# chaiyujin/sdfa-2019

Hardware: AMD Instinct MI355X
Metric: animation frames/s/node (10 s@16 kHz clips); max|Δdgrad| vs CPU ref (higher is better)
Workload: dtype f32

## Files before the change

sdfa-2019_amd/csrc/api_core.cpp:

```cpp
#include "../../include/sdfa_stream.h"
#include "host.h"

#include <climits>
#include <cstdio>
#include <cstring>
#include <string>

static thread_local std::string g_err;

int sdfa_failv(int code, const char *fmt, va_list ap) {
    char buf[512];
    vsnprintf(buf, sizeof buf, fmt, ap);
    g_err = buf;
    return code;
}

int sdfa_fail(int code, const char *fmt, ...) {
    va_list ap;
    va_start(ap, fmt);
    sdfa_failv(code, fmt, ap);
    va_end(ap);
    return code;
}

thread_local int g_sdfa_mel_fft_radix4 = 0;
thread_local int g_sdfa_gather_plain_order = 0;
thread_local int g_sdfa_frontend_two_kernel = 0;
thread_local int g_sdfa_frontend_stream_block = 0;
thread_local int g_sdfa_frontend_stream_slots = 0;
thread_local int g_sdfa_frontend_stream_spin_max = 0;
thread_local int g_sdfa_frontend_stream_phases = 0;
thread_local int g_sdfa_frontend_t_major = 0;
extern thread_local int g_sdfa_gemm_variant;
thread_local int g_sdfa_freq_lstm_shape = 0;
thread_local int g_sdfa_pca_lds = 0;
thread_local int g_sdfa_pca_fp32 = 0;
thread_local int g_sdfa_conv_fp32 = 0;
thread_local int g_sdfa_time_lstm_split = 0;
thread_local int g_sdfa_time_lstm_fuse_x = 0;
thread_local int g_sdfa_time_lstm_handoff = 0;
thread_local int g_sdfa_time_lstm_timeout_us = 0;
thread_local int g_sdfa_share_gx0_off = 0;
thread_local int g_sdfa_encoder_dedup_off = 0;
thread_local int g_sdfa_share_hash_bits = 0;
thread_local int g_sdfa_freq_proj_tail = 0;
thread_local int g_sdfa_attn_unfused = 0;

extern "C" {

int sdfa_abi_version(void) { return SDFA_ABI_VERSION; }
int sdfa_stream_abi_version(void) { return SDFA_STREAM_ABI_VERSION; }
const char *sdfa_last_error(void) { return g_err.c_str(); }

int sdfa_debug_set_option(const char *name, int value) {
    struct Option { const char *name; int *var; int lo = INT_MIN, hi = INT_MAX; const char *accepts = nullptr; };
    thread_local const Option options[] = {
        {"attn_unfused", &g_sdfa_attn_unfused},
        {"share_gx0_off", &g_sdfa_share_gx0_off},
        {"encoder_dedup_off", &g_sdfa_encoder_dedup_off},
        {"share_hash_bits", &g_sdfa_share_hash_bits, 0, 32, "0 (the whole hash) or 1..32 low bits"},
        {"freq_proj_tail", &g_sdfa_freq_proj_tail, 0, 2, "0 (rule), 1 (never) or 2 (always)"},
        {"frontend_two_kernel", &g_sdfa_frontend_two_kernel},
        {"frontend_stream_phases", &g_sdfa_frontend_stream_phases},
        {"frontend_stream_spin_max", &g_sdfa_frontend_stream_spin_max, 0, INT_MAX, "0 (default) or a positive poll count"},
        {"frontend_stream_block", &g_sdfa_frontend_stream_block, 0, 256, "0 (default) or 1..256 frames"},
        {"frontend_stream_slots", &g_sdfa_frontend_stream_slots, 0, 256, "0 (default) or 1..256 workgroups per block"},
        {"gather_plain_order", &g_sdfa_gather_plain_order},
        {"mel_fft_radix4", &g_sdfa_mel_fft_radix4},
        {"frontend_t_major", &g_sdfa_frontend_t_major},
        {"time_lstm_timeout_us", &g_sdfa_time_lstm_timeout_us},
        {"time_lstm_handoff", &g_sdfa_time_lstm_handoff},
        {"time_lstm_split", &g_sdfa_time_lstm_split},
        {"time_lstm_fuse_x", &g_sdfa_time_lstm_fuse_x, 0, 3, "0 (rule), 1 (never), 2 or 3 (always, 32- / 64-frame tiles)"},
        {"gemm_variant", &g_sdfa_gemm_variant},
        {"freq_lstm_shape", &g_sdfa_freq_lstm_shape},
        {"pca_lds", &g_sdfa_pca_lds},
        {"conv_fp32", &g_sdfa_conv_fp32},
        {"pca_fp32", &g_sdfa_pca_fp32},
    };
    for (const Option &o : options)
        if (name && !strcmp(name, o.name)) {
            if (value < o.lo || value > o.hi) return sdfa_fail(SDFA_EINVAL, "%s: %s", o.name, o.accepts);
            *o.var = value;
            return SDFA_OK;
        }
    return sdfa_fail(SDFA_EINVAL, "unknown option '%s'", name ? name : "(null)");
}

}
```

sdfa-2019_amd/csrc/api_forward.cpp:

```cpp
#include "common.h"
#include "host.h"
#include "kernels.h"
#include "model.h"

#include <algorithm>

extern thread_local int g_sdfa_gemm_variant, g_sdfa_freq_lstm_shape, g_sdfa_pca_lds, g_sdfa_pca_fp32, g_sdfa_conv_fp32, g_sdfa_share_gx0_off, g_sdfa_attn_unfused, g_sdfa_encoder_dedup_off,
    g_sdfa_freq_proj_tail, g_sdfa_share_hash_bits;

namespace {

constexpr int64_t CT_WORDS = 2048, CT_FLAGS = 16, ST_WORDS = SDFA_WS_STATUS_BYTES / 4;

struct Ws {
    int64_t P1, X3, HF, Z, GX, H0, H1, KP, QC, QP, ZK, SH, ZU, total;
    int64_t TRUNK, A0, A1, COEF;
    int64_t CT_FREQ, CT_PCA, CT_FLAG;
};

Ws layout(int64_t Nc, bool keep) {
    const int64_t Mc = 64 * Nc;
    Ws w{};
    int64_t o = 0;
    auto take = [&](int64_t n) { int64_t r = o; o += round_up(n, 64); return r; };
    take(ST_WORDS);
    if (keep) {
        w.P1 = take(2048 * Mc); w.X3 = take(2048 * Mc); w.HF = take((int64_t)HF_SLAB_ROWS * 4 * Mc); w.Z = take(256 * Mc);
        w.GX = take(2048 * Mc); w.H0 = take(512 * Mc); w.H1 = take(512 * Mc); w.KP = take(128 * Mc);
    } else {
        const int64_t A = take(2048 * Mc);
        const int64_t B = take(2048 * Mc);
        w.HF = take((int64_t)HF_SLAB_ROWS * 4 * Mc);
        w.P1 = A; w.GX = A;
        w.X3 = B; w.Z = B; w.H0 = B + 256 * Mc; w.H1 = B + 768 * Mc; w.KP = B + 1280 * Mc;
    }
    w.QC = take(512 * Nc); w.QP = take(128 * Nc); w.ZK = take(512 * Nc);
    const int64_t R = take(2560 * Nc);
    w.TRUNK = R; w.A0 = R + 512 * Nc; w.A1 = R + 1024 * Nc; w.COEF = R + 1280 * Nc;
    w.SH = take(sdfa_share_table_words(Nc) + 111);
    w.ZU = keep ? take(256 * Mc) : w.P1;
    const int64_t CT = take(CT_WORDS);
    w.CT_FREQ = CT; w.CT_PCA = CT + 1; w.CT_FLAG = CT + CT_FLAGS;
    w.total = o;
    return w;
}

int64_t capacity(int64_t bytes, bool keep) {
    const int64_t per128 = layout(128, keep).total * 4;
    int64_t nc = (bytes / per128 + 2) * 128;
    while (nc > 0 && layout(nc, keep).total * 4 > bytes) nc -= 128;
    return nc;
}

struct Prof {
    const sdfa_model *m;
    hipStream_t s;
    hipEvent_t pending = nullptr;
    void begin(const char *stage) {
        if (!m->profile) return;
        sdfa_model::Ev e; e.stage = stage;
        (void)hipEventCreate(&e.a); (void)hipEventCreate(&e.b);
        (void)hipEventRecord(e.a, s);
        pending = e.b;
        std::lock_guard<std::mutex> lk(m->ev_mu);
        m->events.push_back(e);
    }
    void end() {
        if (!m->profile || !pending) return;
        (void)hipEventRecord(pending, s);
        pending = nullptr;
    }
};

GemmArgs gemm_fc(const sdfa_model::Fc &fc, const float *Q, int64_t ldq, float *D, int64_t Nc, const int64_t *spk, int64_t nreal) {
    GemmArgs g = sdfa_gemm_k4(fc.w, fc.Ppad, Q, ldq, D, Nc, fc.K);
    g.bias = fc.b; g.cond_w = fc.cw; g.cond_idx = fc.cw ? spk : nullptr;
    g.Pstore = fc.Pstore; g.Qreal = nreal; g.act = fc.act;
    return g;
}

}

extern "C" {

int64_t sdfa_workspace_bytes(const sdfa_model *m, int64_t max_frames) {
    if (!m || max_frames <= 0) return sdfa_fail(SDFA_EINVAL, "workspace_bytes: bad argument");
    return layout(round_up(max_frames, 128), m->keep).total * 4;
}

int sdfa_debug_keep_intermediates(sdfa_model *m, int on) {
    if (!m) return sdfa_fail(SDFA_EINVAL, "null model");
    m->keep = on != 0;
    return SDFA_OK;
}

int sdfa_profile_enable(sdfa_model *m, int on) {
    if (!m) return sdfa_fail(SDFA_EINVAL, "null model");
    std::lock_guard<std::mutex> lk(m->ev_mu);
    m->profile = on != 0;
    for (auto &e : m->events) { (void)hipEventDestroy(e.a); (void)hipEventDestroy(e.b); }
    m->events.clear();
    return SDFA_OK;
}

float sdfa_profile_ms(const sdfa_model *m, const char *stage) {
    if (!m || !stage) return (float)sdfa_fail(SDFA_EINVAL, "profile_ms: bad argument");
    float total = 0.f;
    bool any = false;
    std::lock_guard<std::mutex> lk(m->ev_mu);
    for (auto &e : m->events)
        if (e.stage == stage) {
            float ms = 0.f;
            if (hipEventSynchronize(e.b) != hipSuccess || hipEventElapsedTime(&ms, e.a, e.b) != hipSuccess)
                return (float)sdfa_fail(SDFA_EHIP, "profile_ms: event query failed");
            total += ms; any = true;
        }
    return any ? total : (float)sdfa_fail(SDFA_EINVAL, "profile_ms: no such stage '%s'", stage);
}

int sdfa_profile_reset(sdfa_model *m) { return m ? sdfa_profile_enable(m, m->profile) : sdfa_fail(SDFA_EINVAL, "null model"); }

enum { STAGE_BODY = 0, STAGE_ATTENTION = 1, STAGE_REGRESSOR = 2 };
static int stage_terms(const sdfa_model *m, int stage) {
    switch (m->precision) {
    case SDFA_PREC_BF16_ATTENTION: return stage == STAGE_ATTENTION ? 1 : 0;
    case SDFA_PREC_BF16X3_ATTENTION: return stage == STAGE_ATTENTION ? 3 : 0;
    case SDFA_PREC_BF16X6: return 6;
    case SDFA_PREC_BF16X3: return 3;
    case SDFA_PREC_BF16: return 1;
    default: return 0;
    }
}

int sdfa_model_set_precision(sdfa_model *m, int mode) {
    if (!m) return sdfa_fail(SDFA_EINVAL, "null model");
    if (mode < SDFA_PREC_FP32 || mode > SDFA_PREC_BF16X6) return sdfa_fail(SDFA_EINVAL, "unknown precision mode %d", mode);
    m->precision = mode;
    return SDFA_OK;
}

int sdfa_model_precision(const sdfa_model *m) { return m ? m->precision : SDFA_EINVAL; }

int sdfa_model_set_reserved_cus(sdfa_model *m, int k) {
    if (!m) return sdfa_fail(SDFA_EINVAL, "null model");
    if (k < 0 || k > 128) return sdfa_fail(SDFA_EINVAL, "reserved_cus must be in [0, 128], got %d", k);
    m->reserved_cus.store(k);
    return SDFA_OK;
}

static int encoder_impl(const sdfa_model *m, const float *d_audio_feat, int64_t n_frames, const int32_t *d_frame_clip,
                        const int64_t *d_frame_start, int hop, float *d_z, float *d_align, void *d_workspace,
                        int64_t workspace_bytes, void *stream) {
    if (!m || !m->finalized) return sdfa_fail(SDFA_ESTATE, "encoder_forward: model not finalised");
    if (n_frames == 0) return SDFA_OK;
    if (!d_audio_feat || !d_z || !d_workspace || n_frames < 0) return sdfa_fail(SDFA_EINVAL, "encoder_forward: bad argument");
    if (((uintptr_t)d_workspace | (uintptr_t)d_audio_feat | (uintptr_t)d_z) & 15) return sdfa_fail(SDFA_EINVAL, "encoder_forward: pointers must be 16-byte aligned");
    if ((uintptr_t)d_align & 3) return sdfa_fail(SDFA_EINVAL, "encoder_forward: d_align must be 4-byte aligned");
    const int64_t cap = capacity(workspace_bytes, m->keep);
    if (cap < 128) return sdfa_fail(SDFA_ENOSPACE, "encoder_forward: workspace of %lld bytes holds no 128-frame chunk", (long long)workspace_bytes);
    hipStream_t s = (hipStream_t)stream;
    Prof pf{m, s};
    float *ws = (float *)d_workspace;
    for (int64_t f0 = 0; f0 < n_frames; f0 += cap) {
        const int64_t N = std::min(cap, n_frames - f0);
        const int64_t Nc = round_up(N, 128), Mc = 64 * Nc;
        const Ws w = layout(Nc, m->keep);
        ConvArgs ca{};
        ca.audio_feat = d_audio_feat + f0 * (64 * 128 * 3); ca.N = N; ca.Nc = Nc; ca.Mc = Mc;
        ca.w1 = m->w1; ca.b1 = m->b1; ca.s1 = m->s1; ca.t1 = m->t1; ca.P1 = ws + w.P1;
        ca.w2 = m->w2; ca.b2 = m->b2; ca.s2 = m->s2; ca.t2 = m->t2;
        ca.w3 = m->w3; ca.b3 = m->b3; ca.s3 = m->s3; ca.t3 = m->t3; ca.X3 = ws + w.X3;
        const bool table = d_frame_clip != nullptr;
        const bool share = table || (!m->keep && !g_sdfa_encoder_dedup_off);
        const int64_t *d_ulimit = nullptr;
        int32_t *col_to_u = nullptr;
        bool split_tail = false;
        int64_t fat_grid = 0;
        const int64_t *d_qfull = nullptr;
        if (share) {
            ShareArgs sa{};
            sa.N = N; sa.Nc = Nc; sa.Mc = Mc;
            sdfa_share_carve(sa, reinterpret_cast<int32_t *>(ws + w.SH));
            split_tail = !m->keep && stage_terms(m, STAGE_BODY) == 0 && g_sdfa_gemm_variant == 0 && Mc / 256 >= 512 && g_sdfa_freq_proj_tail != 1;
            if (split_tail) {
                fat_grid = sdfa_fat_grid(256, Mc, sdfa_cu_count(), m->reserved_cus.load());
                sa.fat_grid = (int)fat_grid; sa.tail_mode = g_sdfa_freq_proj_tail;
            }
            pf.begin("share_map");
            if (table) {
                sa.frame_clip = d_frame_clip + f0; sa.frame_start = d_frame_start + f0; sa.hop = hop;
                sa.t_lo = 6; sa.t_hi = 58;
                HIP_TRY(sdfa_launch_share_map(sa, s));
            } else {
                sa.feat = ca.audio_feat;
                sa.hash = reinterpret_cast<uint64_t *>(ws + w.HF);
                sa.group_slots = sdfa_share_group_slots(N);
                sa.group_key = sa.hash + Mc; sa.group_first = reinterpret_cast<uint32_t *>(sa.group_key + sa.group_slots);
                sa.hash_bits = g_sdfa_share_hash_bits;
                HIP_TRY(sdfa_launch_share_map_content(sa, s));
            }
            pf.end();
            d_ulimit = sa.counts + 1; d_qfull = sa.counts + 2; col_to_u = sa.col_to_u;
            ca.col_src = sa.col_src; ca.col_limit = d_ulimit;
        }
        const int conv_terms = g_sdfa_conv_fp32 ? 0 : stage_terms(m, STAGE_BODY);
        if (m->keep && conv_terms) {
            pf.begin("conv1"); HIP_TRY(sdfa_launch_conv1(ca, s)); pf.end();
            ca.wb = m->cv_wb; ca.terms = conv_terms;
            pf.begin("conv23"); HIP_TRY(sdfa_launch_conv123(ca, s)); pf.end();
        } else if (m->keep) {
            pf.begin("conv1"); HIP_TRY(sdfa_launch_conv1(ca, s)); pf.end();
            pf.begin("conv23"); HIP_TRY(sdfa_launch_conv23(ca, s)); pf.end();
        } else {
            ca.wb = m->cv_wb; ca.terms = conv_terms;
            pf.begin("conv23"); HIP_TRY(sdfa_launch_conv123(ca, s)); pf.end();
        }

        const int fl_terms = stage_terms(m, STAGE_BODY);
        FreqLstmArgs fa{ws + w.X3, m->fl_w, m->fl_b, ws + w.HF, Mc, d_ulimit, m->fl_wb, fl_terms, reinterpret_cast<int *>(ws + w.CT_FREQ),
                        g_sdfa_freq_lstm_shape ? g_sdfa_freq_lstm_shape : (fl_terms ? 0 : m->freq_shape.load()), m->reserved_cus.load()};
        pf.begin("freq_lstm"); HIP_TRY(sdfa_launch_freq_lstm(fa, s)); pf.end();

        GemmArgs g = sdfa_gemm_k4(m->fp_w, 256, ws + w.HF, Mc, ws + w.Z, Mc, 8192);
        g.bias = m->fp_b; g.q_tile_major = 1; g.q_slab_rows = HF_SLAB_ROWS;
        g.terms = stage_terms(m, STAGE_BODY);
        g.reserve_cus = m->reserved_cus.load();
        if (share) { g.D = ws + w.ZU; g.q_limit = split_tail ? d_qfull : d_ulimit; }
        pf.begin("freq_proj");
        HIP_TRY(sdfa_launch_gemm(g, s));
        if (split_tail) {
            GemmTailArgs gt{m->fp_w, ws + w.HF, m->fp_b, ws + w.ZU, Mc, HF_SLAB_ROWS, d_qfull, d_ulimit, (int)fat_grid - 1};
            HIP_TRY(sdfa_launch_gemm_tail(gt, s));
        }
        pf.end();
        const bool share_gx0 = share && !m->keep && stage_terms(m, STAGE_BODY) == 0 && !g_sdfa_share_gx0_off;
        if (share && !share_gx0) {
            pf.begin("share_expand"); HIP_TRY(sdfa_launch_expand_cols(ws + w.ZU, col_to_u, ws + w.Z, 64, Mc, s)); pf.end();
        }

        const float *xin = share_gx0 ? ws + w.ZU : ws + w.Z;
        float *hout[2] = {ws + w.H0, ws + w.H1};
        const char *gxn[2] = {"gx0", "gx1"}, *lsn[2] = {"lstm0", "lstm1"};
        for (int l = 0; l < 2; ++l) {
            const bool mapped = share_gx0 && l == 0;
            float *gx = mapped ? ws + w.HF : ws + w.GX;
            GemmArgs gi = sdfa_gemm_k4(m->gx_w[l], 2048, xin, Mc, gx, Mc, l == 0 ? 256 : 512);
            gi.terms = stage_terms(m, STAGE_BODY);
            gi.reserve_cus = m->reserved_cus.load();
            if (mapped) gi.q_limit = d_ulimit;
            TimeLstmArgs ta{gx, m->tl_w[l], hout[l], Nc, Mc, m->tl_wb[l], stage_terms(m, STAGE_BODY),
                            reinterpret_cast<unsigned *>(ws + w.CT_FLAG), CT_WORDS - CT_FLAGS, m->tl_w16[l],
                            reinterpret_cast<unsigned *>(ws), m->reserved_cus.load(), mapped ? col_to_u : nullptr};
            if (l == 1 && !m->keep) { ta.X = xin; ta.Wxh = m->tl_wxh1; }
            pf.begin(gxn[l]);
            if (!sdfa_time_lstm_fuses_x(ta)) HIP_TRY(sdfa_launch_gemm(gi, s));
            pf.end();
            pf.begin(lsn[l]); HIP_TRY(sdfa_launch_time_lstm(ta, s)); pf.end();
            xin = hout[l];
        }
        const int at_terms = stage_terms(m, STAGE_ATTENTION);
        const bool key_fused = g_sdfa_attn_unfused != 1;
        pf.begin("attn_proj");
        GemmArgs gk = sdfa_gemm_k4(m->kp_w, 128, ws + w.H1, Mc, ws + w.KP, Mc, 512);
        gk.terms = at_terms;
        if (!key_fused) HIP_TRY(sdfa_launch_gemm(gk, s));
        GemmArgs gc = sdfa_gemm_k4(m->qc_w, 512, ws + w.H1 + 31 * Nc * 4, Mc, ws + w.QC, Nc, 1536);
        gc.seg_k = 512; gc.seg_col = Nc; gc.terms = at_terms;
        HIP_TRY(sdfa_launch_gemm(gc, s));
        GemmArgs gq = sdfa_gemm_k4(m->qp_w, 128, ws + w.QC, Nc, ws + w.QP, Nc, 512);
        gq.terms = at_terms;
        HIP_TRY(sdfa_launch_gemm(gq, s));
        const bool tail_fused = key_fused && (at_terms == 0 || at_terms == 6) && g_sdfa_attn_unfused != 2 && sdfa_attn_fuses_tail(Nc, m->reserved_cus.load());
        if (key_fused) {
            AttnKeyArgs ak{};
            ak.Wk = m->kp_w; ak.H = ws + w.H1; ak.QP = ws + w.QP; ak.v = m->at_v; ak.b = m->at_b;
            ak.S = ws + w.KP;
            ak.Nc = Nc; ak.Mc = Mc; ak.terms = at_terms == 6 ? 0 : at_terms; ak.reserve_cus = m->reserved_cus.load();
            if (tail_fused) {
                ak.fuse_tail = 1; ak.Zk4 = ws + w.ZK; ak.z_out = d_z + f0 * 512; ak.align_out = d_align ? d_align + f0 * 64 : nullptr; ak.N = N;
            }
            HIP_TRY(sdfa_launch_attn_key_score(ak, s));
        }
        pf.end();

        AttnArgs aa{};
        aa.KP = ws + w.KP; aa.QP = ws + w.QP; aa.H = ws + w.H1; aa.v = m->at_v; aa.b = m->at_b;
        aa.Zk4 = ws + w.ZK; aa.z_out = d_z + f0 * 512; aa.align_out = d_align ? d_align + f0 * 64 : nullptr;
        aa.N = N; aa.Nc = Nc; aa.Mc = Mc;
        aa.S = key_fused ? ws + w.KP : nullptr;
        pf.begin("attn"); if (!tail_fused) HIP_TRY(sdfa_launch_attn(aa, s)); pf.end();
    }
    return SDFA_OK;
}

int sdfa_model_autotune(sdfa_model *m, int64_t n_frames, void *d_workspace, int64_t workspace_bytes, void *stream) {
    if (!m || !m->finalized) return sdfa_fail(SDFA_ESTATE, "autotune: model not finalised");
    if (!d_workspace || n_frames <= 0 || ((uintptr_t)d_workspace & 15)) return sdfa_fail(SDFA_EINVAL, "autotune: bad argument");
    const int64_t cap = capacity(workspace_bytes, m->keep);
    if (cap < 128) return sdfa_fail(SDFA_ENOSPACE, "autotune: workspace too small");
    const int64_t Nc = round_up(std::min(cap, n_frames), 128), Mc = 64 * Nc;
    const Ws w = layout(Nc, m->keep);
    float *ws = (float *)d_workspace;
    hipStream_t s = (hipStream_t)stream;
    HIP_TRY(hipMemsetAsync(ws + w.X3, 0, (size_t)2048 * Mc * sizeof(float), s));
    hipEvent_t e0, e1;
    HIP_TRY(hipEventCreate(&e0));
    HIP_TRY(hipEventCreate(&e1));
    static const int forms[] = {9, 8, 5, 3};
    float best_ms = 0.f;
    int best = m->freq_shape.load(), rc = SDFA_OK;
    for (int form : forms) {
        FreqLstmArgs fa{ws + w.X3, m->fl_w, m->fl_b, ws + w.HF, Mc, nullptr, m->fl_wb, 0, reinterpret_cast<int *>(ws + w.CT_FREQ), form, m->reserved_cus.load()};
        float ms = 0.f;
        for (int rep = 0; rep < 3 && rc == SDFA_OK; ++rep) {
            if (rep == 1 && hipEventRecord(e0, s) != hipSuccess) rc = SDFA_EHIP;
            if (sdfa_launch_freq_lstm(fa, s) != hipSuccess) rc = SDFA_EHIP;
        }
        if (rc == SDFA_OK && (hipEventRecord(e1, s) != hipSuccess || hipEventSynchronize(e1) != hipSuccess || hipEventElapsedTime(&ms, e0, e1) != hipSuccess)) rc = SDFA_EHIP;
        if (rc != SDFA_OK) break;
        if (best_ms == 0.f || ms < best_ms) { best_ms = ms; best = form; }
    }
    (void)hipEventDestroy(e0);
    (void)hipEventDestroy(e1);
    if (rc != SDFA_OK) return sdfa_fail(rc, "autotune: a HIP call failed: %s", hipGetErrorString(hipGetLastError()));
    m->freq_shape.store(best);
    return best;
}

int sdfa_encoder_forward(const sdfa_model *m, const float *d_audio_feat, int64_t n_frames, float *d_z, float *d_align,
                         void *d_workspace, int64_t workspace_bytes, void *stream) {
    return encoder_impl(m, d_audio_feat, n_frames, nullptr, nullptr, 0, d_z, d_align, d_workspace, workspace_bytes, stream);
}

int sdfa_encoder_forward_shared(const sdfa_model *m, const float *d_audio_feat, int64_t n_frames, const int32_t *d_frame_clip,
                                const int64_t *d_frame_start, int hop, float *d_z, float *d_align, void *d_workspace,
                                int64_t workspace_bytes, void *stream) {
    if (!d_frame_clip || !d_frame_start || hop <= 0) return sdfa_fail(SDFA_EINVAL, "encoder_forward_shared: frame table missing");
    return encoder_impl(m, d_audio_feat, n_frames, d_frame_clip, d_frame_start, hop, d_z, d_align, d_workspace, workspace_bytes, stream);
}

static hipError_t expand_rows(const sdfa_model *m, const float *coef, int64_t N, int64_t Nc, int64_t f0,
                              float *const *h_d_outs, int n_outs, int *queue, hipStream_t s) {
    float *d_out = h_d_outs[0];
    if (m->pca_n == 2) {
        PcaArgs pa{};
        pa.coef = coef; pa.basis_s = m->pca_q[0]; pa.basis_r = m->pca_q[1]; pa.mean_s = m->pca_bias[0]; pa.mean_r = m->pca_bias[1];
        pa.out = d_out + f0 * m->out_dim; pa.N = N; pa.Nc = Nc; pa.out_dim = m->out_dim;
        pa.n_extra = n_outs - 1;
        pa.reserve_cus = m->reserved_cus.load();
        pa.basis_b = m->pca_qb; pa.terms = (g_sdfa_pca_fp32 || m->precision != SDFA_PREC_BF16X3) ? 0 : 3;
        for (int x = 1; x < n_outs; ++x) pa.out_extra[x - 1] = h_d_outs[x] + f0 * m->out_dim;
// ... 162 lines not shown
```

sdfa-2019_amd/csrc/kernels.h:

```cpp
#pragma once
#include <hip/hip_runtime.h>
#include <stdint.h>

enum { ACT_NONE = 0, ACT_LRELU = 1, ACT_TANH = 2 };

constexpr int HF_SLAB_ROWS = 2048;
enum { OUT_K4 = 0, OUT_ROW = 1 };
constexpr int SDFA_MAX_DESTS = 8;

struct GemmArgs {
    const float *P;
    const float *Q;
    float *D;
    const float *bias;
    const float *cond_w;
    const int64_t *cond_idx;
    int64_t ldp, ldq, ldd;
    int64_t Ppad, Qpad;
    int64_t Pstore;
    int64_t Qreal;
    int K;
    int seg_k;
    int64_t seg_col;
    int act, out_mode, bias_on_q;
// ... 12 lines not shown
    g.P = P; g.Q = Q; g.D = D;
    g.ldp = rows; g.Ppad = rows; g.Pstore = rows;
    g.ldq = ldq; g.ldd = cols; g.Qpad = cols; g.Qreal = cols;
    g.K = K; g.seg_k = K; g.act = ACT_NONE; g.out_mode = OUT_K4;
    return g;
}

struct PcaArgs {
    const float *coef;
    const float *basis_s, *basis_r;
    const float *mean_s, *mean_r;
    float *out;
    int64_t N, Nc, out_dim, ld_s, ld_r, cols_s, cols_r;
    float *out_extra[SDFA_MAX_DESTS - 1];
    int n_extra;
    int reserve_cus;
    const void *basis_b;
    int terms;
};
hipError_t sdfa_launch_pca_dgrad(const PcaArgs &a, hipStream_t s);
hipError_t sdfa_launch_pca_dgrad_res(const PcaArgs &a, int *queue, hipStream_t s);

struct FrontendConsts {
    const float *hamm;
    const float2 *twiddle;
    const int *mel_bin0;
    const float *mel_w8;
    int win, hop, sliding, nbins_used, nnz;
};
hipError_t sdfa_launch_frontend(const FrontendConsts &c, const float *pcm, const int64_t *clip_off,
                                const int64_t *clip_len, const int32_t *frame_clip, const int64_t *frame_start,
                                int64_t n_frames, float *audio_feat, hipStream_t s);
hipError_t sdfa_launch_mel_columns(const FrontendConsts &c, const float *pcm, const int64_t *clip_off, const int64_t *clip_len,
                                   const int32_t *frame_clip, const int64_t *frame_start, const int32_t *col_src,
                                   const int64_t *n_distinct, float *mel_table, hipStream_t s);
hipError_t sdfa_launch_mel_stream(const FrontendConsts &c, const float *pcm, const int64_t *clip_off, const int64_t *clip_len,
                                  const int32_t *frame_clip, const int64_t *frame_start, const int32_t *prev, const int32_t *shift,
                                  int64_t n_frames, int block, int slots, int producer_consumer, int spin_max, int *status, float *audio_feat, hipStream_t s);
hipError_t sdfa_launch_mel_ring(const FrontendConsts &c, const float *rings, int r, int n_rings, const int64_t *view_ring, const int64_t *view_hi,
                                const int32_t *frame_view, const int64_t *frame_start, const int32_t *prev, const int32_t *shift, int64_t n_frames,
                                int block, int slots, int producer_consumer, int spin_max, int *status, float *audio_feat, hipStream_t s);
hipError_t sdfa_launch_ring_append(float *rings, int r, int n_rings, const int64_t *seg, int n_seg, const float *src, int64_t n_src, hipStream_t s);
hipError_t sdfa_launch_gather_features(const float *mel_table, const int32_t *col_to_u, int64_t n_frames, int64_t Nc, int frame_major,
                                       float *audio_feat, hipStream_t s);

struct ConvArgs {
    const float *audio_feat;
    int64_t N, Nc, Mc;
    const float *w1, *b1, *s1, *t1;
    float *P1;
    const float *w2, *b2, *s2, *t2;
    const float *w3, *b3, *s3, *t3;
    float *X3;
    const int32_t *col_src;
    const int64_t *col_limit;
    const void *wb;
    int terms;
};
hipError_t sdfa_launch_conv1(const ConvArgs &a, hipStream_t s);
hipError_t sdfa_launch_conv23(const ConvArgs &a, hipStream_t s);
hipError_t sdfa_launch_conv123(const ConvArgs &a, hipStream_t s);

struct FreqLstmArgs {
    const float *X3;
    const float *W;
    const float *bias;
    float *HF;
    int64_t Mc;
    const int64_t *col_limit;
    const void *Wb;
    int terms;
    int *tile_counter;
    int shape;
    int reserve_cus;
};
hipError_t sdfa_launch_freq_lstm(const FreqLstmArgs &a, hipStream_t s);

struct TimeLstmArgs {
    const float *GX;
    const float *W;
    float *H;
    int64_t Nc, Mc;
    const void *Wb;
    int terms;
    unsigned *flags;
    int64_t flag_words;
    const float *W16;
    unsigned *status;
    int reserve_cus;
    const int32_t *col_map;
    const float *X = nullptr;
    const float *Wxh = nullptr;
};
hipError_t sdfa_launch_time_lstm(const TimeLstmArgs &a, hipStream_t s);
int sdfa_time_lstm_fuses_x(const TimeLstmArgs &a);

struct AttnArgs {
    const float *KP;
    const float *QP;
    const float *H;
    const float *v;
    const float *b;
    float *Zk4;
    float *z_out;
    float *align_out;
    int64_t N, Nc, Mc;
    const float *S;
};
hipError_t sdfa_launch_attn(const AttnArgs &a, hipStream_t s);

struct AttnKeyArgs {
    const float *Wk;
    const float *H;
    const float *QP;
    const float *v, *b;
    float *S;
    int64_t Nc, Mc;
    int terms;
    int reserve_cus;
    int ts_shift;
    int fuse_tail;
    float *Zk4, *z_out, *align_out;
    int64_t N;
};
bool sdfa_attn_fuses_tail(int64_t Nc, int reserve_cus);
hipError_t sdfa_launch_attn_key_score(const AttnKeyArgs &a, hipStream_t s);

hipError_t sdfa_launch_rows_to_k4(const float *src, int64_t N, int F, float *dst, int64_t ld, hipStream_t s);
hipError_t sdfa_launch_rows_seg_to_k4(const float *src, int64_t src_ld, int64_t N, int c0, int nf, float *dst, int64_t ld,
                                      int f0, int nf_pad, hipStream_t s);
hipError_t sdfa_launch_k4_to_rows(const float *src, int64_t ld, int64_t N, int F, int f0, int nf, float *dst,
                                  int64_t dst_ld, hipStream_t s);
hipError_t sdfa_launch_tap(const float *src, int what, int64_t N, int64_t Nc, float *dst, hipStream_t s);

struct ShareArgs {
    const int32_t *frame_clip;
    const int64_t *frame_start;
    int hop;
    int t_lo, t_hi;
    int frame_major;
    int64_t N, Nc, Mc;
    int32_t *prev, *shift;
    int32_t *owner, *flag, *uid;
    int32_t *tile_sum;
    int32_t *col_src;
    int32_t *col_to_u;
    int64_t *counts;
    const float *feat;
    uint64_t *hash;
    uint64_t *group_key;
    uint32_t *group_first;
    int64_t group_slots;
    int hash_bits;
    int fat_grid;
    int tail_mode;
};
inline int64_t sdfa_share_table_words(int64_t Nc) { return 16 + 2 * Nc + 5 * (64 * Nc) + (64 * Nc) / 1024 + 1; }
inline int64_t sdfa_share_group_slots(int64_t N) { int64_t s = 1024; while (s < 2 * 64 * N) s <<= 1; return s; }
inline void sdfa_share_carve(ShareArgs &a, int32_t *base) {
    a.counts = reinterpret_cast<int64_t *>(base);
    a.prev = base + 16; a.shift = a.prev + a.Nc;
    a.owner = a.shift + a.Nc; a.flag = a.owner + a.Mc; a.uid = a.flag + a.Mc;
    a.col_src = a.uid + a.Mc; a.col_to_u = a.col_src + a.Mc; a.tile_sum = a.col_to_u + a.Mc;
}
hipError_t sdfa_launch_share_map(const ShareArgs &a, hipStream_t s);
hipError_t sdfa_launch_share_map_content(const ShareArgs &a, hipStream_t s);
hipError_t sdfa_launch_share_prev(const ShareArgs &a, hipStream_t s);
hipError_t sdfa_launch_expand_cols(const float *Zu, const int32_t *col_to_u, float *Z, int nquads, int64_t Mc, hipStream_t s);

struct GemmTailArgs {
    const float *P, *Q, *bias;
    float *D;
    int64_t ldd;
    int q_slab_rows;
    const int64_t *q_lo, *q_hi;
    int max_tiles;
};
hipError_t sdfa_launch_gemm_tail(const GemmTailArgs &a, hipStream_t s);
inline int64_t sdfa_fat_grid(int64_t rows, int64_t cols, int cus, int reserve_cus) {
    const int64_t ntiles = (rows / 256) * (cols / 256), wgs = cus - reserve_cus > 1 ? cus - reserve_cus : 1;
    return ntiles < wgs ? ntiles : wgs;
}

struct MeshArgs {
    const float *dgrad;
    int64_t n_frames;
    int n_tris, n_verts, n_free, free_pad;
    int n_src_tris;
    const int64_t *seek_src;
    const float *seek_w;
    const float *reg_xt;
    const int *inc_ptr;
    const int *inc_tri;
    const float *inc_coef;
    const int *vert_col;
    const float *tmpl;
    float *rhs;
    const float *sol;
    float *verts;
    int64_t ld;
};
hipError_t sdfa_launch_mesh_rhs(const MeshArgs &a, hipStream_t s);
hipError_t sdfa_launch_mesh_scatter(const MeshArgs &a, hipStream_t s);
hipError_t sdfa_launch_seek_plan(const int32_t *tslist, const int64_t *frame_off, const int64_t *query_off, int n_clips, double fps,
                                 int64_t n_queries, int64_t *src, float *w, hipStream_t s);
hipError_t sdfa_launch_seek_rows(const float *rows, int64_t width, const int64_t *src, const float *w, int64_t nq, float *out, hipStream_t s);
struct DgradArgs {
    const float *src;
    const float *target;
    const uint32_t *faces;
    const uint8_t *mask;
    int64_t n_frames;
    int n_tris, n_verts, target_is_offsets;
    double eps;
    float *out32;
    double *out64;
};
hipError_t sdfa_launch_deform_grad(const DgradArgs &a, hipStream_t s);
hipError_t sdfa_launch_ensemble_mean(const float *a, const float *b, int64_t n, float *out, hipStream_t s);

struct ResampleArgs {
    const float *x;
    int64_t n_in;
    float *y;
    int64_t n_res, n_out;
    const double *win, *delta;
    const double *treg;
    int64_t nwin, step;
    double scale;
    int num_table;
};
hipError_t sdfa_launch_resample(const ResampleArgs &a, hipStream_t s);
constexpr int STREAM_RING_MIRROR = 2048;
constexpr int STREAM_MAX_RATES = 8;
struct StreamRate {
    const double *win;
    int64_t step;
    double scale;
};
struct StreamResampleArgs {
    const float *in_rings;
    float *rings;
    int r_in, n_in_rings, r, n_rings;
    const int64_t *seg;
    const double *treg;
    int64_t n_treg, nwin;
    int num_table, n_rates;
    StreamRate rate[STREAM_MAX_RATES];
};
hipError_t sdfa_launch_stream_resample(const StreamResampleArgs &a, int n_seg, int64_t max_count, hipStream_t s);
```

sdfa-2019_amd/csrc/share.hip:

```cpp
#include "common.h"
#include "kernels.h"

namespace {


__global__ void share_prev_kernel(ShareArgs a) {
    const int64_t n = (int64_t)blockIdx.x * blockDim.x + threadIdx.x;
    if (n >= a.Nc) return;
    int prev = -1, shift = 0;
    if (n < a.N) {
        const int clip = a.frame_clip[n];
        const int64_t s = a.frame_start[n];
        for (int back = 1; back <= 64 && n - back >= 0; ++back) {
            const int64_t q = n - back;
            if (a.frame_clip[q] != clip) break;
            const int64_t diff = s - a.frame_start[q];
            if (diff <= 0) break;
            if (diff > (int64_t)(a.t_hi - a.t_lo) * a.hop) break;
            if (diff % a.hop == 0) { prev = (int)q; shift = (int)(diff / a.hop); break; }
        }
    }
    a.prev[n] = prev;
    a.shift[n] = shift;
}

__device__ __forceinline__ int64_t col_index(const ShareArgs &a, int64_t n, int t) { return a.frame_major ? n * 64 + t : (int64_t)t * a.Nc + n; }
__device__ __forceinline__ void col_of(const ShareArgs &a, int64_t i, int64_t &n, int &t) {
    if (a.frame_major) { n = i >> 6; t = (int)(i & 63); } else { n = i % a.Nc; t = (int)(i / a.Nc); }
}

__global__ void share_owner_kernel(ShareArgs a) {
    const int64_t i = (int64_t)blockIdx.x * blockDim.x + threadIdx.x;
    if (i >= a.Mc) return;
    int64_t n;
    int t;
    col_of(a, i, n, t);
    if (n >= a.N) { a.owner[i] = -1; a.flag[i] = 0; return; }
    while (t >= a.t_lo && t <= a.t_hi) {
        const int p = a.prev[n];
        if (p < 0) break;
        const int tt = t + a.shift[n];
        if (tt > a.t_hi) break;
        n = p; t = tt;
    }
    const int64_t o = col_index(a, n, t);
    a.owner[i] = (int)o;
    a.flag[i] = o == i ? 1 : 0;
}

constexpr int COL_QUADS = 96;
constexpr unsigned long long GROUP_EMPTY = ~0ull;

__device__ __forceinline__ uint64_t mix64(uint64_t x) {
    x ^= x >> 32; x *= 0xd6e8feb86659fd93ull;
    x ^= x >> 32; x *= 0xd6e8feb86659fd93ull;
    return x ^ (x >> 32);
}

__global__ __launch_bounds__(256) void share_hash_kernel(ShareArgs a) {
    const int l = threadIdx.x & 31;
    const int64_t col = ((int64_t)blockIdx.x * 256 + threadIdx.x) >> 5, M = a.N * 64;
    uint64_t h = 0;
    if (col < M) {
        const uint4 *row = reinterpret_cast<const uint4 *>(a.feat) + col * COL_QUADS;
#pragma unroll
        for (int j = 0; j < 3; ++j) {
            const int q = l + 32 * j;
            const uint4 v = row[q];
            const uint64_t lo = (uint64_t)v.x | (uint64_t)v.y << 32, hi = (uint64_t)v.z | (uint64_t)v.w << 32;
            h += mix64(lo + 0x9e3779b97f4a7c15ull * (uint64_t)(2 * q + 1)) + mix64(hi + 0x9e3779b97f4a7c15ull * (uint64_t)(2 * q + 2));
        }
    }
    for (int off = 16; off; off >>= 1) h += __shfl_xor(h, off);
    h = mix64(h);
    if (a.hash_bits) h &= (1ull << a.hash_bits) - 1;
    h |= 1;
    __shared__ unsigned long long wg_hash[8];
    const int c = threadIdx.x >> 5;
    if (l == 0) { a.hash[col] = h; wg_hash[c] = h; }
    __syncthreads();
    if (l) return;
    for (int j = 0; j < c; ++j)
        if (wg_hash[j] == h) return;
    const unsigned long long key = ~h;
    const unsigned i = (unsigned)col_index(a, col >> 6, (int)(col & 63));
    unsigned long long *keys = reinterpret_cast<unsigned long long *>(a.group_key);
    const int64_t mask = a.group_slots - 1;
    for (int64_t slot = (int64_t)(h >> 1) & mask, k = 0; k <= mask; ++k, slot = (slot + 1) & mask) {
        unsigned long long cur = __hip_atomic_load(&keys[slot], __ATOMIC_RELAXED, __HIP_MEMORY_SCOPE_AGENT);
        if (cur == GROUP_EMPTY) {
            cur = atomicCAS(&keys[slot], GROUP_EMPTY, key);
            if (cur == GROUP_EMPTY) cur = key;
        }
        if (cur != key) continue;
        if (__hip_atomic_load(&a.group_first[slot], __ATOMIC_RELAXED, __HIP_MEMORY_SCOPE_AGENT) > i) atomicMin(&a.group_first[slot], i);
        break;
    }
}

__global__ __launch_bounds__(256) void share_resolve_kernel(ShareArgs a) {
    const int l = threadIdx.x & 31, half = (threadIdx.x & 63) >> 5;
    const int64_t col = ((int64_t)blockIdx.x * 256 + threadIdx.x) >> 5, n = col >> 6;
    const int64_t i = col_index(a, n, (int)(col & 63));
    if (n >= a.N) {
        if (l == 0) { a.owner[i] = -1; a.flag[i] = 0; }
        return;
    }
    const uint64_t h = a.hash[col], mask = (uint64_t)a.group_slots - 1;
    uint64_t slot = (h >> 1) & mask;
    for (uint64_t k = 0; k < mask && a.group_key[slot] != ~h; ++k) slot = (slot + 1) & mask;
    const int64_t cand = a.group_key[slot] == ~h ? (int64_t)a.group_first[slot] : i;
    bool differ = false;
    if (cand != i) {
        int64_t cn;
        int ct;
        col_of(a, cand, cn, ct);
        const uint4 *x = reinterpret_cast<const uint4 *>(a.feat) + col * COL_QUADS, *y = reinterpret_cast<const uint4 *>(a.feat) + (cn * 64 + ct) * COL_QUADS;
#pragma unroll
        for (int k = 0; k < 3; ++k) {
            const uint4 u = x[l + 32 * k], v = y[l + 32 * k];
            differ |= ((u.x ^ v.x) | (u.y ^ v.y) | (u.z ^ v.z) | (u.w ^ v.w)) != 0;
        }
    }
    const uint64_t bad = __ballot(differ) >> (32 * half) & 0xffffffffull;
    if (l == 0) {
        const int64_t o = bad ? i : cand;
        a.owner[i] = (int)o;
        a.flag[i] = o == i ? 1 : 0;
    }
}

__device__ __forceinline__ int block_inclusive_scan_1024(int v, int *part) {
    const int tid = threadIdx.x;
    part[tid] = v;
    __syncthreads();
    for (int off = 1; off < 1024; off <<= 1) {
        const int x = tid >= off ? part[tid - off] : 0;
        __syncthreads();
        part[tid] += x;
        __syncthreads();
    }
    return part[tid];
}

__global__ __launch_bounds__(1024) void share_scan_tiles_kernel(ShareArgs a) {
    __shared__ int part[1024];
    const int64_t i = (int64_t)blockIdx.x * 1024 + threadIdx.x;
    const int f = i < a.Mc ? a.flag[i] : 0;
    const int inc = block_inclusive_scan_1024(f, part);
    if (i < a.Mc) a.uid[i] = inc - f;
    if (threadIdx.x == 1023) a.tile_sum[blockIdx.x] = inc;
}

constexpr int TAIL_NUM = 3, TAIL_DEN = 4;
__global__ __launch_bounds__(1024) void share_scan_sums_kernel(ShareArgs a, int ntiles) {
    __shared__ int part[1024];
    int carry = 0;
    for (int base = 0; base < ntiles; base += 1024) {
        const int t = base + threadIdx.x;
        const int v = t < ntiles ? a.tile_sum[t] : 0;
        const int inc = block_inclusive_scan_1024(v, part);
        if (t < ntiles) a.tile_sum[t] = carry + inc - v;
        carry += part[1023];
        __syncthreads();
    }
    if (threadIdx.x == 0) {
        const int64_t mu = carry, pad = (mu + 255) / 256 * 256;
        a.counts[0] = mu;
        a.counts[1] = pad;
        int64_t q_full = pad;
        if (a.fat_grid > 0 && a.tail_mode != 1) {
            const int64_t T = pad / 256, G = a.fat_grid, r = T % G;
            if (a.tail_mode == 2 || r * TAIL_DEN <= G * TAIL_NUM) q_full = (T - r) * 256;
        }
        a.counts[2] = q_full;
    }
}

__global__ __launch_bounds__(1024) void share_scan_fix_kernel(ShareArgs a) {
    const int64_t i = (int64_t)blockIdx.x * 1024 + threadIdx.x;
    const int64_t mu = a.counts[0], pad = a.counts[1];
    if (i < a.Mc) {
        const int u = a.uid[i] + a.tile_sum[blockIdx.x];
        a.uid[i] = u;
        int64_t n;
        int t;
        col_of(a, i, n, t);
        if (a.flag[i]) a.col_src[u] = (int)(n * 64 + t);
    }
    if (i >= mu && i < pad) a.col_src[i] = -1;
}

__global__ void share_assign_kernel(ShareArgs a) {
    const int64_t m = (int64_t)blockIdx.x * blockDim.x + threadIdx.x;
    if (m >= a.Mc) return;
    const int o = a.owner[m];
    a.col_to_u[m] = o >= 0 ? a.uid[o] : 0;
}

__global__ void expand_cols_kernel(const float4 *__restrict__ Zu, const int32_t *__restrict__ col_to_u, float4 *__restrict__ Z,
                                   int nquads, int64_t Mc) {
    const int64_t m = (int64_t)blockIdx.x * blockDim.x + threadIdx.x;
    if (m >= Mc) return;
    const int64_t u = col_to_u[m];
    for (int q = 0; q < nquads; ++q) Z[(int64_t)q * Mc + m] = Zu[(int64_t)q * Mc + u];
}

}

static void launch_share_numbering(const ShareArgs &a, hipStream_t s) {
    const int ntiles = (int)((a.Mc + 1023) / 1024);
    hipLaunchKernelGGL(share_scan_tiles_kernel, dim3(ntiles), dim3(1024), 0, s, a);
    hipLaunchKernelGGL(share_scan_sums_kernel, dim3(1), dim3(1024), 0, s, a, ntiles);
    hipLaunchKernelGGL(share_scan_fix_kernel, dim3(ntiles), dim3(1024), 0, s, a);
    hipLaunchKernelGGL(share_assign_kernel, dim3((unsigned)((a.Mc + 255) / 256)), dim3(256), 0, s, a);
}

hipError_t sdfa_launch_share_map_content(const ShareArgs &a, hipStream_t s) {
    const hipError_t e = hipMemsetAsync(a.group_key, 0xff, (size_t)a.group_slots * 12, s);
    if (e != hipSuccess) return e;
    hipLaunchKernelGGL(share_hash_kernel, dim3((unsigned)(a.N * 8)), dim3(256), 0, s, a);
    hipLaunchKernelGGL(share_resolve_kernel, dim3((unsigned)(a.Nc * 8)), dim3(256), 0, s, a);
    launch_share_numbering(a, s);
    return hipGetLastError();
}

hipError_t sdfa_launch_share_map(const ShareArgs &a, hipStream_t s) {
    hipLaunchKernelGGL(share_prev_kernel, dim3((unsigned)((a.Nc + 255) / 256)), dim3(256), 0, s, a);
    hipLaunchKernelGGL(share_owner_kernel, dim3((unsigned)((a.Mc + 255) / 256)), dim3(256), 0, s, a);
    launch_share_numbering(a, s);
    return hipGetLastError();
}

hipError_t sdfa_launch_share_prev(const ShareArgs &a, hipStream_t s) {
    hipLaunchKernelGGL(share_prev_kernel, dim3((unsigned)((a.Nc + 255) / 256)), dim3(256), 0, s, a);
    return hipGetLastError();
}

hipError_t sdfa_launch_expand_cols(const float *Zu, const int32_t *col_to_u, float *Z, int nquads, int64_t Mc, hipStream_t s) {
    hipLaunchKernelGGL(expand_cols_kernel, dim3((unsigned)((Mc + 255) / 256)), dim3(256), 0, s,
                       reinterpret_cast<const float4 *>(Zu), col_to_u, reinterpret_cast<float4 *>(Z), nquads, Mc);
    return hipGetLastError();
}
```

Baseline: 151,000.

## Verify column equality at hash insert to skip feature comparisons in resolve

Adds a default content-dedup path in which the hash kernel inserts each column into the group table and immediately compares its features against the current group representative. It records per-column verification and per-slot dispute flags. The resolve kernel then only re-compares columns whose slot was disputed or unverified, compacting that work into a per-block list. The aim is to avoid a second full feature read in the resolve pass. The cost is extra atomics and a larger table memset, and correctness depends on the group_first min-race handling and on the workspace having room for the new disputed and verified arrays.

```diff
diff --git a/sdfa-2019_amd/csrc/api_core.cpp b/sdfa-2019_amd/csrc/api_core.cpp
--- a/sdfa-2019_amd/csrc/api_core.cpp
+++ b/sdfa-2019_amd/csrc/api_core.cpp
@@ -43,6 +43,7 @@
 thread_local int g_sdfa_share_gx0_off = 0;
 thread_local int g_sdfa_encoder_dedup_off = 0;
 thread_local int g_sdfa_share_hash_bits = 0;
+thread_local int g_sdfa_share_scan = 0;
 thread_local int g_sdfa_freq_proj_tail = 0;
 thread_local int g_sdfa_attn_unfused = 0;
 
@@ -59,6 +60,7 @@
         {"share_gx0_off", &g_sdfa_share_gx0_off},
         {"encoder_dedup_off", &g_sdfa_encoder_dedup_off},
         {"share_hash_bits", &g_sdfa_share_hash_bits, 0, 32, "0 (the whole hash) or 1..32 low bits"},
+        {"share_scan", &g_sdfa_share_scan, 0, 1, "0 (verify at insert) or 1 (hash pass + resolve pass)"},
         {"freq_proj_tail", &g_sdfa_freq_proj_tail, 0, 2, "0 (rule), 1 (never) or 2 (always)"},
         {"frontend_two_kernel", &g_sdfa_frontend_two_kernel},
         {"frontend_stream_phases", &g_sdfa_frontend_stream_phases},
diff --git a/sdfa-2019_amd/csrc/api_forward.cpp b/sdfa-2019_amd/csrc/api_forward.cpp
--- a/sdfa-2019_amd/csrc/api_forward.cpp
+++ b/sdfa-2019_amd/csrc/api_forward.cpp
@@ -6,7 +6,7 @@
 #include <algorithm>
 
 extern thread_local int g_sdfa_gemm_variant, g_sdfa_freq_lstm_shape, g_sdfa_pca_lds, g_sdfa_pca_fp32, g_sdfa_conv_fp32, g_sdfa_share_gx0_off, g_sdfa_attn_unfused, g_sdfa_encoder_dedup_off,
-    g_sdfa_freq_proj_tail, g_sdfa_share_hash_bits;
+    g_sdfa_freq_proj_tail, g_sdfa_share_hash_bits, g_sdfa_share_scan;
 
 namespace {
 
@@ -196,7 +196,8 @@
                 sa.hash = reinterpret_cast<uint64_t *>(ws + w.HF);
                 sa.group_slots = sdfa_share_group_slots(N);
                 sa.group_key = sa.hash + Mc; sa.group_first = reinterpret_cast<uint32_t *>(sa.group_key + sa.group_slots);
-                sa.hash_bits = g_sdfa_share_hash_bits;
+                sa.disputed = sa.group_first + sa.group_slots; sa.verified = reinterpret_cast<uint8_t *>(sa.disputed + sa.group_slots);
+                sa.hash_bits = g_sdfa_share_hash_bits; sa.scan_form = g_sdfa_share_scan;
                 HIP_TRY(sdfa_launch_share_map_content(sa, s));
             }
             pf.end();
diff --git a/sdfa-2019_amd/csrc/kernels.h b/sdfa-2019_amd/csrc/kernels.h
--- a/sdfa-2019_amd/csrc/kernels.h
+++ b/sdfa-2019_amd/csrc/kernels.h
@@ -188,6 +188,9 @@
     uint32_t *group_first;
     int64_t group_slots;
     int hash_bits;
+    uint32_t *disputed;
+    uint8_t *verified;
+    int scan_form;
     int fat_grid;
     int tail_mode;
 };
diff --git a/sdfa-2019_amd/csrc/share.hip b/sdfa-2019_amd/csrc/share.hip
--- a/sdfa-2019_amd/csrc/share.hip
+++ b/sdfa-2019_amd/csrc/share.hip
@@ -130,6 +130,131 @@
     }
 }
 
+constexpr unsigned FIRST_EMPTY = ~0u, UNDISPUTED = ~0u;
+
+__device__ __forceinline__ uint64_t quad_hash(const uint4 v, int q) {
+    const uint64_t lo = (uint64_t)v.x | (uint64_t)v.y << 32, hi = (uint64_t)v.z | (uint64_t)v.w << 32;
+    return mix64(lo + 0x9e3779b97f4a7c15ull * (uint64_t)(2 * q + 1)) + mix64(hi + 0x9e3779b97f4a7c15ull * (uint64_t)(2 * q + 2));
+}
+__device__ __forceinline__ bool quads_differ(const uint4 u, const uint4 v) { return ((u.x ^ v.x) | (u.y ^ v.y) | (u.z ^ v.z) | (u.w ^ v.w)) != 0; }
+
+__device__ __forceinline__ int64_t table_slot(unsigned long long *keys, int64_t mask, uint64_t h, unsigned long long cur) {
+    const unsigned long long key = ~h;
+    int64_t slot = (int64_t)(h >> 1) & mask;
+    for (int64_t k = 0; k <= mask; ++k) {
+        if (cur == GROUP_EMPTY) {
+            cur = atomicCAS(&keys[slot], GROUP_EMPTY, key);
+            if (cur == GROUP_EMPTY) cur = key;
+        }
+        if (cur == key) return slot;
+        slot = (slot + 1) & mask;
+        cur = __hip_atomic_load(&keys[slot], __ATOMIC_RELAXED, __HIP_MEMORY_SCOPE_AGENT);
+    }
+    return -1;
+}
+
+__global__ __launch_bounds__(256) void share_hash_verify_kernel(ShareArgs a) {
+    const int l = threadIdx.x & 31, c = threadIdx.x >> 5, half = c & 1;
+    const int64_t col = (int64_t)blockIdx.x * 8 + c, mask = a.group_slots - 1;
+    const uint4 *feat = reinterpret_cast<const uint4 *>(a.feat), *row = feat + col * COL_QUADS + l;
+    const uint4 q0 = row[0], q1 = row[32], q2 = row[64];
+    uint64_t h = quad_hash(q0, l) + quad_hash(q1, l + 32) + quad_hash(q2, l + 64);
+    for (int off = 16; off; off >>= 1) h += __shfl_xor(h, off);
+    h = mix64(h);
+    if (a.hash_bits) h &= (1ull << a.hash_bits) - 1;
+    h |= 1;
+    __shared__ unsigned long long wg_hash[8];
+    if (l == 0) { a.hash[col] = h; wg_hash[c] = h; }
+    __syncthreads();
+    int lead = c;
+    for (int j = c - 1; j >= 0; --j)
+        if (wg_hash[j] == h) lead = j;
+    unsigned long long *keys = reinterpret_cast<unsigned long long *>(a.group_key);
+    const int64_t home = (int64_t)(h >> 1) & mask;
+    const unsigned i = (unsigned)col_index(a, col >> 6, (int)(col & 63));
+    int64_t slot = -1;
+    int other = lead < c ? (int)(col - (c - lead)) : -1;
+    bool root = false;
+    if (l == 0 && lead == c) {
+        const unsigned long long seen = __hip_atomic_load(&keys[home], __ATOMIC_RELAXED, __HIP_MEMORY_SCOPE_AGENT);
+        unsigned cand = __hip_atomic_load(&a.group_first[home], __ATOMIC_RELAXED, __HIP_MEMORY_SCOPE_AGENT);
+        if (seen != ~h) cand = FIRST_EMPTY;
+        slot = table_slot(keys, mask, h, seen);
+        if (slot >= 0) {
+            if (slot != home) cand = __hip_atomic_load(&a.group_first[slot], __ATOMIC_RELAXED, __HIP_MEMORY_SCOPE_AGENT);
+            if (cand == FIRST_EMPTY) {
+                cand = atomicMin(&a.group_first[slot], i);
+                root = cand == FIRST_EMPTY;
+            } else if (cand > i) {
+                atomicMin(&a.group_first[slot], i);
+            }
+            if (!root && cand != i && cand < (unsigned)a.Mc) {
+                const unsigned cn = a.frame_major ? cand >> 6 : cand % (unsigned)a.Nc, ct = a.frame_major ? cand & 63 : cand / (unsigned)a.Nc;
+                if (cn < a.N) other = (int)(cn * 64 + ct);
+            }
+        }
+    }
+    other = __shfl(other, threadIdx.x & 32);
+    bool differ = false;
+    if (other >= 0) {
+        const uint4 *y = feat + (int64_t)other * COL_QUADS + l;
+        differ = (int)quads_differ(q0, y[0]) | (int)quads_differ(q1, y[32]) | (int)quads_differ(q2, y[64]);
+    }
+    const uint64_t bad = __ballot(differ) >> (32 * half) & 0xffffffffull;
+    if (l) return;
+    const bool ok = root || (other >= 0 && !bad);
+    a.verified[col] = ok ? 1 : 0;
+    if (ok) return;
+    if (lead < c) slot = table_slot(keys, mask, h, __hip_atomic_load(&keys[home], __ATOMIC_RELAXED, __HIP_MEMORY_SCOPE_AGENT));
+    if (slot >= 0) a.disputed[slot] = 1;
+}
+
+__global__ __launch_bounds__(256) void share_resolve_verified_kernel(ShareArgs a) {
+    __shared__ int todo_col[256], todo_cand[256], ntodo;
+    if (threadIdx.x == 0) ntodo = 0;
+    __syncthreads();
+    const int64_t base = (int64_t)blockIdx.x * 256, col = base + threadIdx.x, n = col >> 6;
+    const int64_t i = col_index(a, n, (int)(col & 63));
+    if (n >= a.N) {
+        a.owner[i] = -1; a.flag[i] = 0;
+    } else {
+        const uint64_t h = a.hash[col], mask = (uint64_t)a.group_slots - 1;
+        uint64_t slot = (h >> 1) & mask;
+        for (uint64_t k = 0; k < mask && a.group_key[slot] != ~h; ++k) slot = (slot + 1) & mask;
+        const bool found = a.group_key[slot] == ~h && a.group_first[slot] != FIRST_EMPTY;
+        const int64_t cand = found ? (int64_t)a.group_first[slot] : i;
+        if (cand == i || (found && a.disputed[slot] == UNDISPUTED && a.verified[col])) {
+            a.owner[i] = (int)cand; a.flag[i] = cand == i ? 1 : 0;
+        } else {
+            const int k = atomicAdd(&ntodo, 1);
+            todo_col[k] = threadIdx.x; todo_cand[k] = (int)cand;
+        }
+    }
+    __syncthreads();
+    const int l = threadIdx.x & 31, half = (threadIdx.x & 63) >> 5, count = ntodo;
+    for (int k0 = (threadIdx.x >> 6) * 2; k0 < count; k0 += 8) {
+        const int k = k0 + half;
+        const bool live = k < count;
+        bool differ = false;
+        int64_t mine = 0, cand = 0;
+        if (live) {
+            mine = base + todo_col[k]; cand = todo_cand[k];
+            int64_t cn;
+            int ct;
+            col_of(a, cand, cn, ct);
+            const uint4 *x = reinterpret_cast<const uint4 *>(a.feat) + mine * COL_QUADS, *y = reinterpret_cast<const uint4 *>(a.feat) + (cn * 64 + ct) * COL_QUADS;
+#pragma unroll
+            for (int j = 0; j < 3; ++j) differ |= (int)quads_differ(x[l + 32 * j], y[l + 32 * j]);
+        }
+        const uint64_t bad = __ballot(differ) >> (32 * half) & 0xffffffffull;
+        if (live && l == 0) {
+            const int64_t mi = col_index(a, mine >> 6, (int)(mine & 63)), o = bad ? mi : cand;
+            a.owner[mi] = (int)o;
+            a.flag[mi] = o == mi ? 1 : 0;
+        }
+    }
+}
+
 __device__ __forceinline__ int block_inclusive_scan_1024(int v, int *part) {
     const int tid = threadIdx.x;
     part[tid] = v;
@@ -217,10 +342,15 @@
 }
 
 hipError_t sdfa_launch_share_map_content(const ShareArgs &a, hipStream_t s) {
-    const hipError_t e = hipMemsetAsync(a.group_key, 0xff, (size_t)a.group_slots * 12, s);
+    const hipError_t e = hipMemsetAsync(a.group_key, 0xff, (size_t)a.group_slots * (a.scan_form == 1 ? 12 : 16), s);
     if (e != hipSuccess) return e;
-    hipLaunchKernelGGL(share_hash_kernel, dim3((unsigned)(a.N * 8)), dim3(256), 0, s, a);
-    hipLaunchKernelGGL(share_resolve_kernel, dim3((unsigned)(a.Nc * 8)), dim3(256), 0, s, a);
+    if (a.scan_form == 1) {
+        hipLaunchKernelGGL(share_hash_kernel, dim3((unsigned)(a.N * 8)), dim3(256), 0, s, a);
+        hipLaunchKernelGGL(share_resolve_kernel, dim3((unsigned)(a.Nc * 8)), dim3(256), 0, s, a);
+    } else {
+        hipLaunchKernelGGL(share_hash_verify_kernel, dim3((unsigned)(a.N * 8)), dim3(256), 0, s, a);
+        hipLaunchKernelGGL(share_resolve_verified_kernel, dim3((unsigned)(a.Mc / 256)), dim3(256), 0, s, a);
+    }
     launch_share_numbering(a, s);
     return hipGetLastError();
 }
```

Result: no change. 151,200 (median of 6 runs) (+0.2%).
